# MayeulCassier/Matrix-Factorization-With-Comparison-Data

Measured on AMD Instinct MI355X. Metric: triplet-updates/sec, higher is better.
Workload: dtype f32

## Files before the change

matrix-factorization-with-comparison-data_amd/csrc/resident_kernel.h:

```cpp
#pragma once
#include "common.h"
#include "train_common.h"

namespace mfcd_detail {

typedef unsigned long long u64;

#define MFCD_LAMBDA_INLINE __attribute__((always_inline))

#ifdef MFCD_RES_STATS
#define RS_NOW() ((u64)__builtin_amdgcn_s_memtime())
#define RS_ADD(slot, val) rs_acc[slot] += (u64)(val)
#else
#define RS_NOW() ((u64)0)
#define RS_ADD(slot, val) ((void)0)
#endif

typedef const __attribute__((address_space(4))) float *ScalarTablePtr;
__device__ __forceinline__ StepScalars load_step_scalars(const StepScalars *table, int k)
{
    const ScalarTablePtr f = (ScalarTablePtr)(table + k);
    StepScalars s;
    s.neg_step_size = f[0];
    s.bc2_sqrt = f[1];
    s.inv_bc2_sqrt = f[2];
    s.pad = 0.0f;
    return s;
}


__device__ __forceinline__ u64 pack_granule(unsigned tag, float v)
{
    return ((u64)tag << 32) | (u64)__float_as_uint(v);
}

__device__ __forceinline__ u64 load_granule(const u64 *p)
{
    return __hip_atomic_load(p, __ATOMIC_RELAXED, __HIP_MEMORY_SCOPE_AGENT);
}

__device__ __forceinline__ void store_granule(u64 *p, unsigned tag, float v)
{
    __hip_atomic_store(p, pack_granule(tag, v), __ATOMIC_RELAXED, __HIP_MEMORY_SCOPE_AGENT);
}

struct RowMap {
    int n, m, c;
    __host__ __device__ int vrow_u(int u) const { return u < c ? 2 * u : 2 * c + (u - c); }
    __host__ __device__ int vrow_v(int i) const { return i < c ? 2 * i + 1 : 2 * c + (i - c); }
    __host__ __device__ int users_below(int x) const
    {
        if (x <= 2 * c) return (x + 1) >> 1;
        return n > c ? c + (x - 2 * c) : c;
    }
    __host__ __device__ int items_below(int x) const
    {
        if (x <= 2 * c) return x >> 1;
        return m > c ? c + (x - 2 * c) : c;
    }
    __host__ __device__ bool is_item(int vr) const { return vr < 2 * c ? (vr & 1) != 0 : m > n; }
    __host__ __device__ int table_row(int vr) const { return vr < 2 * c ? vr >> 1 : c + (vr - 2 * c); }
};
__host__ __device__ inline RowMap make_row_map(int n, int m)
{
    RowMap r;
    r.n = n; r.m = m; r.c = n < m ? n : m;
    return r;
}

constexpr int kEventCap = 64;
constexpr unsigned kEventNone = 0xFFFFFFF8u;
constexpr int kEventMaxLocalRows = 1024;

struct ResidentArgs {
    const ResidentCold *cold;
    const mfcd_sample *samples;
    const StepScalars *sc;
    u64 *mailbox;
    void *loss_terms;
    u64 *dbg;
    unsigned tag_base;
    int64_t N;
    int B, n, m, K, NW;
    int lookahead;
    int fast_math;
    int bf16;
    AdamStatic ac;
};

__device__ __forceinline__ mfcd_sample load_record(const mfcd_sample *__restrict__ samples, int64_t pos0, int Bk,
                                                   int base, int lane)
{
    mfcd_sample s;
    s.u = s.i = s.j = -0x40000000;
    s.z = 0.0f;
    if (base + lane < Bk) s = samples[pos0 + base + lane];
    return s;
}

struct Masks {
    u64 mu, mi, mj;
};

template <int D, int Q, int LOOK, bool FAST, bool BF16 = false>
__global__ __launch_bounds__(256) __attribute__((amdgpu_waves_per_eu(Q >= 16 ? 2 : 1)))
void resident_train_kernel(ResidentArgs a)
{
    constexpr int S = D >= 64 ? D / 64 : 1;
    constexpr int RPR = D < 64 ? 64 / D : 1;
    constexpr int EW = 64 * Q;
    static_assert(EW % D == 0, "a wave's slice must hold whole rows");
    static_assert(EW / D <= kEventMaxLocalRows, "local row indices are 10-bit fields of an event entry");
    constexpr bool GRL = Q >= 16;
    extern __shared__ __attribute__((aligned(16))) float lds_dyn[];
    const int lane = threadIdx.x & 63;
    const int gw = blockIdx.x * (blockDim.x >> 6) + (threadIdx.x >> 6);
    if (gw >= a.NW) return;

    const int64_t T = (int64_t)(a.n + a.m) * D;
    const int64_t ebase = (int64_t)gw * EW;
    const int Rlo = (int)(ebase / D);
    const int64_t eend = (ebase + EW < T) ? ebase + EW : T;
    const int Rhi = (int)(eend / D);
    const int lcol = lane & (D - 1);
    auto elem_is_item = [&](int64_t e) MFCD_LAMBDA_INLINE { return make_row_map(a.n, a.m).is_item((int)(e / D)); };
    auto elem_offset = [&](int64_t e) MFCD_LAMBDA_INLINE { return (int64_t)make_row_map(a.n, a.m).table_row((int)(e / D)) * D + (e % D); };

#ifdef MFCD_RES_STATS
    u64 rs_acc[8] = {0, 0, 0, 0, 0, 0, 0, 0};
    const u64 rs_t0 = RS_NOW();
    [[maybe_unused]] const u64 rs_abs_t0 = __builtin_amdgcn_s_memrealtime();
    [[maybe_unused]] u64 rs_abs_l0 = 0, rs_abs_l1 = 0;
    [[maybe_unused]] u64 rs_hit[8] = {0, 0, 0, 0, 0, 0, 0, 0};
    [[maybe_unused]] u64 rs_mark = 0;
#endif
    float p[Q], m1[Q], m2[Q], gr[GRL ? 1 : Q];
    float *const lgr = lds_dyn + (threadIdx.x >> 6) * (GRL ? EW : 0);
    auto post = [](float x) MFCD_LAMBDA_INLINE {
        if constexpr (BF16) return (float)(mfcd_bf16)x;
        else return x;
    };
    {
        const ResidentCold c = *a.cold;
#pragma unroll
        for (int q = 0; q < Q; ++q) {
            const int64_t e = ebase + q * 64 + lane;
            p[q] = m1[q] = m2[q] = 0.0f;
            if constexpr (GRL) lgr[q * 64 + lane] = 0.0f;
            if (e < T) {
                const int64_t o = elem_offset(e);
                if (!elem_is_item(e)) { p[q] = BF16 ? (float)((const mfcd_bf16 *)c.U)[o] : c.U[o]; m1[q] = c.mU[o]; m2[q] = c.vU[o]; }
                else { p[q] = BF16 ? (float)((const mfcd_bf16 *)c.V)[o] : c.V[o]; m1[q] = c.mV[o]; m2[q] = c.vV[o]; }
            }
        }
    }

    auto batch_size = [&](int step) MFCD_LAMBDA_INLINE {
        const int64_t pos0 = (int64_t)step * a.B;
        return (int)((a.N - pos0) < a.B ? (a.N - pos0) : a.B);
    };
    auto scan = [&](const mfcd_sample &s, int Bk, int base) MFCD_LAMBDA_INLINE {
        const bool valid = base + lane < Bk;
        const int ru = s.u, ri = s.i, rj = s.j;
        Masks M;
        M.mu = __ballot(valid && ru >= Rlo && ru < Rhi);
        M.mi = __ballot(valid && ri >= Rlo && ri < Rhi);
        M.mj = __ballot(valid && rj >= Rlo && rj < Rhi);
        return M;
    };
    auto reg_of = [&](int lr) MFCD_LAMBDA_INLINE { return D >= 64 ? lr * S : lr / RPR; };

    auto give_up = [&](int step, int64_t pos, int what) MFCD_LAMBDA_INLINE {
        int *const status = a.cold->status;
        if (lane == 0) {
            if (__hip_atomic_exchange(status, 1, __ATOMIC_RELAXED, __HIP_MEMORY_SCOPE_AGENT) == 0 && a.dbg) {
                a.dbg[0] = (u64)gw; a.dbg[1] = (u64)step; a.dbg[2] = (u64)pos; a.dbg[3] = (u64)what;
            }
        }
    };
    auto poll_failed = [&](unsigned &spins, unsigned &limit) MFCD_LAMBDA_INLINE -> bool {
        if (spins == 0) limit = (unsigned)a.cold->spin_limit;
        ++spins;
        if (spins > limit || (spins & 255u) == 0) {
            if (spins > limit ||
                __hip_atomic_load(a.cold->status, __ATOMIC_RELAXED, __HIP_MEMORY_SCOPE_AGENT) != 0)
                return true;
        }
        return false;
    };

    auto store_row = [&](int lr, int64_t slot, unsigned tag) MFCD_LAMBDA_INLINE {
        u64 *dst = a.mailbox + slot * D;
        const int q0 = reg_of(lr);
#pragma unroll
        for (int q = 0; q < Q; ++q) {
            if (q >= q0 && q < q0 + S) {
                if constexpr (D >= 64) {
                    store_granule(dst + (q - q0) * 64 + lane, tag, p[q]);
                } else {
                    if (lane / D == lr % RPR) store_granule(dst + lcol, tag, p[q]);
                }
            }
        }
    };

    auto process_hit = [&](bool own0, bool own1, bool own2, int lr0, int lr1, int lr2, float zz, int64_t pos,
                           unsigned tag, float inv_batch, int step) MFCD_LAMBDA_INLINE -> bool {
        const bool own[3] = {own0, own1, own2};
        const int lrs[3] = {lr0, lr1, lr2};
        const u64 *slot = a.mailbox + pos * 3 * D;

        float row[3][S];
#pragma unroll
        for (int r = 0; r < 3; ++r) {
#pragma unroll
            for (int s2 = 0; s2 < S; ++s2) row[r][s2] = 0.0f;
            if (!own[r]) continue;
            const int q0 = reg_of(lrs[r]);
            if constexpr (D >= 64) {
#pragma unroll
                for (int q = 0; q < Q; ++q)
                    if (q >= q0 && q < q0 + S) row[r][(q * 64 % D) / 64] = p[q];
            } else {
                float sel = 0.0f;
#pragma unroll
                for (int q = 0; q < Q; ++q) sel = (q == q0) ? p[q] : sel;
                const float v = __shfl(sel, (lrs[r] % RPR) * D + lcol, MFCD_WAVE);
                row[r][0] = lane < D ? v : 0.0f;
            }
        }
        unsigned spins = 0, limit = 0;
        [[maybe_unused]] u64 rs_w0 = 0;
        RS_ADD(4, 1ull);
#ifdef MFCD_RES_STAMPS
        { const u64 t = RS_NOW(); rs_hit[0] += t - rs_mark; rs_mark = t; }
#endif
#if defined(MFCD_RES_STAGGER) && MFCD_RES_STAGGER > 0
        {
            u64 ga[3][S], gb[3][S];
            auto issue = [&](u64 (&g)[3][S]) MFCD_LAMBDA_INLINE {
#pragma unroll
                for (int r = 0; r < 3; ++r) {
                    if (own[r]) continue;
#pragma unroll
                    for (int s2 = 0; s2 < S; ++s2) {
                        const int c = lane + 64 * s2;
                        if (c < D) g[r][s2] = load_granule(slot + (int64_t)r * D + c);
                    }
                }
            };
            auto check = [&](const u64 (&g)[3][S]) MFCD_LAMBDA_INLINE -> bool {
                bool ok = true;
#pragma unroll
                for (int r = 0; r < 3; ++r) {
                    if (own[r]) continue;
#pragma unroll
                    for (int s2 = 0; s2 < S; ++s2) {
                        const int c = lane + 64 * s2;
                        if (c < D) {
                            ok = ok && ((unsigned)(g[r][s2] >> 32) == tag);
                            row[r][s2] = __uint_as_float((unsigned)g[r][s2]);
                        }
                    }
                }
                return __all(ok);
            };
            issue(ga);
            if (!check(ga)) {
#ifdef MFCD_RES_STATS
                rs_w0 = RS_NOW();
#endif
                issue(ga);
                __builtin_amdgcn_s_sleep(MFCD_RES_STAGGER);
                issue(gb);
                while (true) {
                    RS_ADD(5, 1);
                    if (poll_failed(spins, limit)) {
                        give_up(step, pos, (own0 ? 1 : 0) | (own1 ? 2 : 0) | (own2 ? 4 : 0));
                        return false;
                    }
                    if (check(ga)) break;
                    issue(ga);
                    if (check(gb)) break;
                    issue(gb);
                }
            }
        }
#else
        while (true) {
            bool ok = true;
#pragma unroll
            for (int r = 0; r < 3; ++r) {
                if (own[r]) continue;
#pragma unroll
                for (int s2 = 0; s2 < S; ++s2) {
                    const int c = lane + 64 * s2;
                    if (c < D) {
                        const u64 gq = load_granule(slot + (int64_t)r * D + c);
                        ok = ok && ((unsigned)(gq >> 32) == tag);
                        row[r][s2] = __uint_as_float((unsigned)gq);
                    }
                }
            }
            if (__all(ok)) break;
#ifdef MFCD_RES_STATS
            if (spins == 0) rs_w0 = RS_NOW();
            RS_ADD(5, 1);
#endif
            if (poll_failed(spins, limit)) {
                give_up(step, pos, (own0 ? 1 : 0) | (own1 ? 2 : 0) | (own2 ? 4 : 0));
                return false;
            }
        }
#endif
#ifdef MFCD_RES_STATS
        if (spins) RS_ADD(2, RS_NOW() - rs_w0);
        else RS_ADD(4, 1ull << 40);
#endif
#ifdef MFCD_RES_STAMPS
        { const u64 t = RS_NOW(); rs_hit[1] += t - rs_mark; if (!spins) { rs_hit[6] += t - rs_mark; rs_hit[7] += 1; } rs_mark = t; }
#endif

        float acc = 0.0f;
#pragma unroll
        for (int s2 = 0; s2 < S; ++s2) acc += row[0][s2] * (row[1][s2] - row[2][s2]);
        float pr, g;
        if constexpr (FAST) {
            const float x = wave_sum64(acc);
            const float e = __builtin_amdgcn_exp2f(x * -1.44269504088896340736f);
            const float dn = 1.0f + e;
            pr = div_newton(1.0f, dn, __builtin_amdgcn_rcpf(dn));
            pr = (e == __builtin_inff()) ? 0.0f : pr;
            const float den = fmaxf((1.0f - pr) * pr, 1e-12f);
            const float num = inv_batch * (pr - zz);
            g = div_newton(num, den, __builtin_amdgcn_rcpf(den)) * (1.0f - pr) * pr;
        } else {
            pr = sigmoid_f32(wave_sum64(acc));
            g = bce_sigmoid_backward_f32(pr, zz, inv_batch);
        }
        if (own[0] && lane == 0) {
            if constexpr (LOOK > 0) store_granule((u64 *)a.loss_terms + pos, tag, pr);
            else ((float *)a.loss_terms)[pos] = pr;
        }

        float du[S], dv[S];
#pragma unroll
        for (int s2 = 0; s2 < S; ++s2) {
            du[s2] = g * (row[1][s2] - row[2][s2]);
            dv[s2] = g * row[0][s2];
        }
        if constexpr (D < 64) {
            du[0] = __shfl(du[0], lcol, MFCD_WAVE);
            dv[0] = __shfl(dv[0], lcol, MFCD_WAVE);
        }
        if constexpr (GRL) {
#pragma unroll
            for (int r = 0; r < 3; ++r) {
                if (!own[r]) continue;
                const int q0 = reg_of(lrs[r]);
                if constexpr (D >= 64) {
#pragma unroll
                    for (int s2 = 0; s2 < S; ++s2)
                        lgr[(q0 + s2) * 64 + lane] += r == 0 ? du[s2] : (r == 1 ? dv[s2] : -dv[s2]);
                } else {
                    if (lane / D == lrs[r] % RPR) lgr[q0 * 64 + lane] += r == 0 ? du[0] : (r == 1 ? dv[0] : -dv[0]);
                }
            }
        } else {
#pragma unroll
            for (int q = 0; q < Q; ++q) {
                const int rowq = (q * 64 + lane) / D;
                const int sq = D >= 64 ? (q * 64 % D) / 64 : 0;
                if (own[0] && rowq == lrs[0]) gr[q] += du[sq];
                if (own[1] && rowq == lrs[1]) gr[q] += dv[sq];
                if (own[2] && rowq == lrs[2]) gr[q] += -dv[sq];
            }
        }
#ifdef MFCD_RES_STAMPS
        { const u64 t = RS_NOW(); rs_hit[2] += t - rs_mark; rs_mark = t; }
#endif
        return true;
    };

    auto step_update = [&](bool hit, const StepScalars &sc) MFCD_LAMBDA_INLINE {
        if constexpr (GRL) {
            if (hit) {
#pragma unroll
                for (int q = 0; q < Q; ++q) {
                    const float g = lgr[q * 64 + lane];
                    lgr[q * 64 + lane] = 0.0f;
                    adam_update_t<FAST>(p[q], m1[q], m2[q], g, a.ac, sc);
                    p[q] = post(p[q]);
                }
            } else {
#pragma unroll
                for (int q = 0; q < Q; ++q) {
                    adam_update_t<FAST>(p[q], m1[q], m2[q], 0.0f, a.ac, sc);
                    p[q] = post(p[q]);
                }
            }
        } else {
            adam_update_q<FAST, Q, false>(p, m1, m2, gr, a.ac, sc);
            if constexpr (BF16) {
#pragma unroll
                for (int q = 0; q < Q; ++q) p[q] = post(p[q]);
            }
        }
    };

    auto generic_loop = [&]() MFCD_LAMBDA_INLINE -> bool {
        auto publish = [&](int step) MFCD_LAMBDA_INLINE {
            const int64_t pos0 = (int64_t)step * a.B;
            const int Bk = batch_size(step);
            for (int base = 0; base < Bk; base += MFCD_WAVE) {
                const mfcd_sample s = load_record(a.samples, pos0, Bk, base, lane);
                const Masks M = scan(s, Bk, base);
                u64 mask = M.mu | M.mi | M.mj;
                while (mask) {
                    const int tl = __ffsll((long long)mask) - 1;
                    mask &= mask - 1;
                    const int64_t slot0 = (pos0 + base + tl) * 3;
                    if ((M.mu >> tl) & 1ull) store_row(__shfl(s.u, tl, MFCD_WAVE) - Rlo, slot0 + 0, a.tag_base + (unsigned)step + 1u);
                    if ((M.mi >> tl) & 1ull) store_row(__shfl(s.i, tl, MFCD_WAVE) - Rlo, slot0 + 1, a.tag_base + (unsigned)step + 1u);
                    if ((M.mj >> tl) & 1ull) store_row(__shfl(s.j, tl, MFCD_WAVE) - Rlo, slot0 + 2, a.tag_base + (unsigned)step + 1u);
                }
            }
        };
        publish(0);
        for (int k = 0; k < a.K; ++k) {
            const int64_t pos0 = (int64_t)k * a.B;
            const int Bk = batch_size(k);
            const float inv_batch = 1.0f / (float)Bk;
            const StepScalars sc = load_step_scalars(a.sc, k);
            if constexpr (!GRL) {
#pragma unroll
                for (int q = 0; q < Q; ++q) gr[q] = 0.0f;
            }
            bool any_hit = false;
            for (int base = 0; base < Bk; base += MFCD_WAVE) {
                const mfcd_sample s = load_record(a.samples, pos0, Bk, base, lane);
                const Masks M = scan(s, Bk, base);
                u64 mask = M.mu | M.mi | M.mj;
                any_hit = any_hit || mask != 0ull;
                while (mask) {
                    const int tl = __ffsll((long long)mask) - 1;
                    mask &= mask - 1;
                    const int hu = __shfl(s.u, tl, MFCD_WAVE) - Rlo, hi = __shfl(s.i, tl, MFCD_WAVE) - Rlo,
                              hj = __shfl(s.j, tl, MFCD_WAVE) - Rlo;
                    const float hz = __shfl(s.z, tl, MFCD_WAVE);
                    const bool ok = process_hit((bool)((M.mu >> tl) & 1ull), (bool)((M.mi >> tl) & 1ull),
                                                (bool)((M.mj >> tl) & 1ull), hu, hi, hj, hz, pos0 + base + tl,
                                                a.tag_base + (unsigned)k + 1u, inv_batch, k);
                    if (__builtin_amdgcn_readfirstlane((int)!ok)) return false;
                }
            }
            step_update(any_hit, sc);
            if (k + 1 < a.K) publish(k + 1);
        }
        return true;
    };

    bool alive = true;

    if constexpr (LOOK > 0) {
        const int W = __builtin_amdgcn_readfirstlane(a.lookahead);
        const int N32 = (int)a.N;
        const int gws = __builtin_amdgcn_readfirstlane(gw);
        const int tshift = (int)a.cold->tshift;
        const int NCH = ((a.K - 1) >> tshift) + 1;

        bool fits = true;
        {
            const unsigned *cnt = a.cold->ev_cnt + (size_t)gws * (size_t)a.cold->nch_cap;
            for (int c = lane; c < NCH; c += MFCD_WAVE) fits = fits && cnt[c] < (unsigned)kEventCap;
            fits = __all(fits);
        }
        if (!__builtin_amdgcn_readfirstlane((int)fits)) {
            alive = generic_loop();
        } else {
            unsigned ekey = kEventNone, erow = 0u;
            int estep = 0x7FFFFF;
            float ez = 0.0f;
            int chunk_end = 0;

            auto load_chunk = [&](int c) MFCD_LAMBDA_INLINE {
                const ResidentCold *cz = a.cold;
                const size_t li = (size_t)gws * (size_t)cz->nch_cap + (size_t)c;
                const uint4 e = cz->ev_ent[li * kEventCap + lane];
                const unsigned n_raw = cz->ev_cnt[li];
                const unsigned n = (unsigned)__builtin_amdgcn_readfirstlane((int)n_raw);
                const unsigned key = (unsigned)lane < n ? e.x : kEventNone;
                unsigned rank = 0u;
                for (unsigned l = 0; l < n; ++l) {
                    const unsigned kl = (unsigned)__builtin_amdgcn_readlane((int)key, (int)l);
                    rank += kl < key ? 1u : 0u;
                }
                const int dest = (int)((unsigned)lane < n ? rank : (unsigned)lane) << 2;
                ekey = (unsigned)__builtin_amdgcn_ds_permute(dest, (int)key);
                erow = (unsigned)__builtin_amdgcn_ds_permute(dest, (int)e.y);
                ez = __builtin_bit_cast(float, __builtin_amdgcn_ds_permute(dest, (int)e.z));
                estep = (int)(ekey >> 9);
                const int ce = (c + 1) << tshift;
                chunk_end = ce < a.K ? ce : a.K;
            };
            auto step_at = [&](int i) MFCD_LAMBDA_INLINE -> int { return __builtin_amdgcn_readlane(estep, i); };
            auto lanes_in = [](int lo, int hi) MFCD_LAMBDA_INLINE -> u64 { return ((1ull << hi) - 1ull) & ~((1ull << lo) - 1ull); };
            auto rowmask = [&](int lr) MFCD_LAMBDA_INLINE -> u64 {
                const bool t = ((ekey & 1u) && (int)(erow & 1023u) == lr) ||
                               ((ekey & 2u) && (int)((erow >> 10) & 1023u) == lr) ||
                               ((ekey & 4u) && (int)((erow >> 20) & 1023u) == lr);
                return __ballot(t);
            };

            auto publish_entry = [&](int idx, int jbase, int conf_lo, int conf_hi, int touch_lo, int touch_hi,
                                     bool need_touch) MFCD_LAMBDA_INLINE {
                const unsigned key_l = (unsigned)__builtin_amdgcn_readlane((int)ekey, idx);
                const unsigned row_l = (unsigned)__builtin_amdgcn_readlane((int)erow, idx);
                const int ke = (int)(key_l >> 9);
                const int tl = (int)((key_l >> 3) & 63u);
#pragma unroll 1
                for (int r = 0; r < 3; ++r) {
                    if (!((key_l >> r) & 1u)) continue;
                    const int lr = (int)((row_l >> (10 * r)) & 1023u);
                    if (conf_lo < conf_hi || need_touch) {
                        const u64 rm = rowmask(lr);
                        if (rm & lanes_in(conf_lo, conf_hi)) continue;
                        if (need_touch && !(rm & lanes_in(touch_lo, touch_hi))) continue;
                    }
                    const int q0 = reg_of(lr);
                    float pp[S], mm1[S], mm2[S];
#pragma unroll
                    for (int s2 = 0; s2 < S; ++s2) pp[s2] = mm1[s2] = mm2[s2] = 0.0f;
#pragma unroll
                    for (int q = 0; q < Q; ++q) {
                        if (q >= q0 && q < q0 + S) {
                            const int s2 = D >= 64 ? (q * 64 % D) / 64 : 0;
                            pp[s2] = p[q];
                            mm1[s2] = m1[q];
                            mm2[s2] = m2[q];
                        }
                    }
                    StepScalars scb = load_step_scalars(a.sc, jbase + 1);
#pragma unroll 1
                    for (int st = jbase + 1; st < ke; ++st) {
                        const StepScalars scn = load_step_scalars(a.sc, st + 1);
#pragma unroll
                        for (int s2 = 0; s2 < S; ++s2) {
                            adam_update_t<FAST>(pp[s2], mm1[s2], mm2[s2], 0.0f, a.ac, scb);
                            pp[s2] = post(pp[s2]);
                        }
                        scb = scn;
                    }
                    u64 *dst = a.mailbox + (((int64_t)ke * a.B + tl) * 3 + r) * D;
                    const unsigned tag = a.tag_base + (unsigned)ke + 1u;
                    if constexpr (D >= 64) {
#pragma unroll
                        for (int s2 = 0; s2 < S; ++s2) store_granule(dst + s2 * 64 + lane, tag, pp[s2]);
                    } else {
                        if (lane / D == lr % RPR) store_granule(dst + lcol, tag, pp[0]);
                    }
                    RS_ADD(7, 1);
                }
            };
            auto publish_fresh = [&](int jbase, int lo, int hi, int touch_lo, int touch_hi) MFCD_LAMBDA_INLINE {
                if (lo >= hi) return;
                [[maybe_unused]] const u64 rs_p0 = RS_NOW();
                int g0 = lo, gstep = step_at(lo);
                for (int idx = lo; idx < hi; ++idx) {
                    const int st = step_at(idx);
                    if (st != gstep) { g0 = idx; gstep = st; }
                    publish_entry(idx, jbase, lo, g0, touch_lo, touch_hi, jbase >= 0);
                }
                RS_ADD(3, RS_NOW() - rs_p0);
            };
            load_chunk(0);
            int hc = 0, pc = __builtin_popcountll(__ballot(estep < W));
            publish_fresh(-1, 0, pc, 0, 0);
            int nh = step_at(0), np = step_at(pc);
            auto next_event = [&]() MFCD_LAMBDA_INLINE -> int {
                const int cp = np - W;
                const int e = nh < cp ? nh : cp;
                return e < chunk_end ? e : chunk_end;
            };
            int next_evt = next_event();

            ScalarTablePtr scp = (ScalarTablePtr)a.sc;
            auto load_scalars_at = [&](ScalarTablePtr f) MFCD_LAMBDA_INLINE {
                StepScalars x;
                x.neg_step_size = f[0];
                x.bc2_sqrt = f[1];
                x.inv_bc2_sqrt = f[2];
                x.pad = 0.0f;
                return x;
            };
            StepScalars sc_cur = load_scalars_at(scp);
            int chunk = 0;
#ifdef MFCD_RES_STATS
            const u64 rs_l0 = RS_NOW();
            rs_acc[6] = rs_l0 - rs_t0;
            rs_abs_l0 = __builtin_amdgcn_s_memrealtime();
#endif
            int k = 0;
            while (true) {
                const int kq = next_evt < a.K ? next_evt : a.K;
                while (k < kq) {
                    scp += 4;
                    const StepScalars sc_next = load_scalars_at(scp);
                    if constexpr (GRL) {
                        step_update(false, sc_cur);
                    } else {
#pragma unroll
                        for (int q = 0; q < Q; ++q) {
                            adam_update_t<FAST>(p[q], m1[q], m2[q], 0.0f, a.ac, sc_cur);
                            p[q] = post(p[q]);
                        }
                    }
                    sc_cur = sc_next;
                    ++k;
                }
                if (k >= a.K) break;
                scp += 4;
                const StepScalars sc_next = load_scalars_at(scp);
                if constexpr (!GRL) {
#pragma unroll
                    for (int q = 0; q < Q; ++q) gr[q] = 0.0f;
                }
                bool hit = false;
                int h0 = 0;
                {
                    __builtin_amdgcn_s_setprio(3);
                    [[maybe_unused]] const u64 rs_e0 = RS_NOW();
#ifdef MFCD_RES_STAMPS
                    rs_mark = rs_e0;
#endif
                    RS_ADD(7, 1ull << 32);
                    if (k == chunk_end) {
                        load_chunk(++chunk);
                        hc = 0;
                        nh = step_at(0);
                        pc = __builtin_popcountll(__ballot(estep < k + W));
                        np = step_at(pc);
                    }
                    if (np == k + W) {
                        [[maybe_unused]] const u64 rs_p0 = RS_NOW();
                        const int g0 = pc;
                        do {
                            publish_entry(pc, k - 1, hc, g0, 0, 0, false);
                            ++pc;
                            np = step_at(pc);
                        } while (np == k + W);
                        RS_ADD(3, RS_NOW() - rs_p0);
                    }
                    h0 = hc;
                    if (nh == k) {
                        hit = true;
                        const int bk = (N32 - k * a.B) < a.B ? (N32 - k * a.B) : a.B;
                        const float inv_batch = 1.0f / (float)bk;
                        const unsigned tag = a.tag_base + (unsigned)k + 1u;
                        do {
                            const unsigned key_l = (unsigned)__builtin_amdgcn_readlane((int)ekey, hc);
                            const unsigned row_l = (unsigned)__builtin_amdgcn_readlane((int)erow, hc);
                            const float z_l = __builtin_bit_cast(float, __builtin_amdgcn_readlane(__builtin_bit_cast(int, ez), hc));
                            const bool ok = process_hit((bool)(key_l & 1u), (bool)(key_l & 2u), (bool)(key_l & 4u),
                                                        (int)(row_l & 1023u), (int)((row_l >> 10) & 1023u),
                                                        (int)((row_l >> 20) & 1023u), z_l,
                                                        (int64_t)k * a.B + (int)((key_l >> 3) & 63u), tag, inv_batch, k);
                            if (__builtin_amdgcn_readfirstlane((int)!ok)) { alive = false; break; }
                            ++hc;
                            nh = step_at(hc);
                        } while (nh == k);
                        if (!alive) break;
                    }
                    next_evt = next_event();
                    if (!hit) __builtin_amdgcn_s_setprio(0);
                    RS_ADD(1, RS_NOW() - rs_e0);
                }
                step_update(hit, sc_cur);
#ifdef MFCD_RES_STAMPS
                if (hit) { const u64 t = RS_NOW(); rs_hit[3] += t - rs_mark; rs_mark = t; }
#endif
                if (__builtin_expect(hit, 0)) {
                    publish_fresh(k, hc, pc, h0, hc);
                    __builtin_amdgcn_s_setprio(0);
#ifdef MFCD_RES_STAMPS
                    { const u64 t = RS_NOW(); rs_hit[4] += t - rs_mark; rs_hit[5] += 1; }
#endif
                }
                sc_cur = sc_next;
                ++k;
            }
            __builtin_amdgcn_s_setprio(0);
#ifdef MFCD_RES_STATS
            rs_abs_l1 = __builtin_amdgcn_s_memrealtime();
            rs_acc[0] = RS_NOW() - rs_l0;
            rs_acc[6] |= (u64)__builtin_amdgcn_s_getreg((31 << 11) | 4) << 32;
            rs_acc[5] |= (u64)__builtin_amdgcn_s_getreg((31 << 11) | 20) << 32;
            if (lane == 0 && a.dbg)
                for (int x = 0; x < 8; ++x) a.dbg[8 + (int64_t)gw * 8 + x] = rs_acc[x];
#endif
        }

        {
            float *const loss_out = a.cold->loss_out;
            if (loss_out != nullptr) {
                for (int k = gws; k < a.K && alive; k += a.NW) {
                    const int64_t off = (int64_t)k * a.B;
                    const int b = (int)((a.N - off) < a.B ? (a.N - off) : a.B);
                    const unsigned tag = a.tag_base + (unsigned)k + 1u;
                    const float zz = lane < b ? a.samples[off + lane].z : 0.0f;
                    unsigned spins = 0, limit = 0;
                    float pr = 0.0f;
                    while (true) {
                        bool ok = true;
                        if (lane < b) {
                            const u64 gq = load_granule((const u64 *)a.loss_terms + off + lane);
                            ok = (unsigned)(gq >> 32) == tag;
                            pr = __uint_as_float((unsigned)gq);
                        }
                        if (__all(ok)) break;
                        __builtin_amdgcn_s_sleep(8);
                        if (poll_failed(spins, limit)) {
                            give_up(k, off, 8);
                            alive = false;
                            break;
                        }
                    }
                    if (!alive) break;
                    float acc = lane < b ? bce_term_f32(pr, zz) : 0.0f;
                    acc = wave_sum64(acc);
                    if (lane == 0) loss_out[k] = acc / (float)b;
                }
            }
        }
        {
            unsigned *const cnt = a.cold->ev_cnt + (size_t)gws * (size_t)a.cold->nch_cap;
            for (int c = lane; c < NCH; c += MFCD_WAVE) cnt[c] = 0u;
        }
    } else {
        alive = generic_loop();
    }

    const ResidentCold c = *a.cold;
#pragma unroll
    for (int q = 0; q < Q; ++q) {
        const int64_t e = ebase + q * 64 + lane;
        if (e < T) {
            const int64_t o = elem_offset(e);
            if (!elem_is_item(e)) {
                if constexpr (BF16) ((mfcd_bf16 *)c.U)[o] = (mfcd_bf16)p[q];
                else c.U[o] = p[q];
                c.mU[o] = m1[q]; c.vU[o] = m2[q];
            } else {
                if constexpr (BF16) ((mfcd_bf16 *)c.V)[o] = (mfcd_bf16)p[q];
                else c.V[o] = p[q];
                c.mV[o] = m1[q]; c.vV[o] = m2[q];
            }
        }
    }
#ifdef MFCD_RES_STAMPS
    if (lane == 0 && a.dbg) {
        u64 *const o = a.dbg + 8 + (int64_t)gw * 8;
        o[1] = rs_abs_t0; o[2] = rs_abs_l0; o[3] = rs_abs_l1; o[7] = __builtin_amdgcn_s_memrealtime();
        for (int x = 0; x < 8; ++x) o[4096 * 8 + x] = rs_hit[x];
    }
#endif
}

}
```

Before: 92.71 million.

## Prefetch mailbox rows before publishing and split Adam update around publish

Splits hit processing into an early issue step that loads the two foreign mailbox rows and a later finish step, so the mailbox loads are in flight while the wave publishes entries for step k+W. The publish-due-roles computation is rewritten to precompute a per-lane due mask with a cross-lane scan. In the non-GRL path, only the registers touched by the hit are Adam-updated before publishing and the rest afterwards, shortening the critical path to the publish. The costs are more register pressure from holding the prefetched granules, a scalar loop in due_roles, and a more complicated ordering that could be wrong.

```diff
diff --git a/matrix-factorization-with-comparison-data_amd/csrc/resident_kernel.h b/matrix-factorization-with-comparison-data_amd/csrc/resident_kernel.h
--- a/matrix-factorization-with-comparison-data_amd/csrc/resident_kernel.h
+++ b/matrix-factorization-with-comparison-data_amd/csrc/resident_kernel.h
@@ -204,11 +204,46 @@
         }
     };
 
-    auto process_hit = [&](bool own0, bool own1, bool own2, int lr0, int lr1, int lr2, float zz, int64_t pos,
-                           unsigned tag, float inv_batch, int step) MFCD_LAMBDA_INLINE -> bool {
-        const bool own[3] = {own0, own1, own2};
-        const int lrs[3] = {lr0, lr1, lr2};
-        const u64 *slot = a.mailbox + pos * 3 * D;
+    struct Hit {
+        bool own[3];
+        int lr[3];
+        float z;
+        int64_t pos;
+        int fa, fb, nf;
+        u64 ga[S], gb[S];
+    };
+    auto issue_look = [&](Hit &h) MFCD_LAMBDA_INLINE {
+        if (h.nf == 0) return;
+        const u64 *slot = a.mailbox + h.pos * 3 * D;
+#pragma unroll
+        for (int s2 = 0; s2 < S; ++s2) {
+            const int c = lane + 64 * s2;
+            h.ga[s2] = h.gb[s2] = 0ull;
+            if (c < D) {
+                h.ga[s2] = load_granule(slot + (int64_t)h.fa * D + c);
+                h.gb[s2] = load_granule(slot + (int64_t)h.fb * D + c);
+            }
+        }
+    };
+    auto make_hit = [&](bool own0, bool own1, bool own2, int lr0, int lr1, int lr2, float zz, int64_t pos) MFCD_LAMBDA_INLINE {
+        Hit h;
+        h.own[0] = own0; h.own[1] = own1; h.own[2] = own2;
+        h.lr[0] = lr0; h.lr[1] = lr1; h.lr[2] = lr2;
+        h.z = zz;
+        h.pos = pos;
+        h.fa = !own0 ? 0 : (!own1 ? 1 : 2);
+        h.fb = !own2 ? 2 : (!own1 ? 1 : 0);
+        h.nf = (own0 ? 0 : 1) + (own1 ? 0 : 1) + (own2 ? 0 : 1);
+        issue_look(h);
+        return h;
+    };
+
+    [[maybe_unused]] unsigned touched_q = 0u;
+    auto finish_hit = [&](Hit &h, unsigned tag, float inv_batch, int step) MFCD_LAMBDA_INLINE -> bool {
+        const bool(&own)[3] = h.own;
+        const int(&lrs)[3] = h.lr;
+        const float zz = h.z;
+        const int64_t pos = h.pos;
 
         float row[3][S];
 #pragma unroll
@@ -235,84 +270,40 @@
 #ifdef MFCD_RES_STAMPS
         { const u64 t = RS_NOW(); rs_hit[0] += t - rs_mark; rs_mark = t; }
 #endif
-#if defined(MFCD_RES_STAGGER) && MFCD_RES_STAGGER > 0
-        {
-            u64 ga[3][S], gb[3][S];
-            auto issue = [&](u64 (&g)[3][S]) MFCD_LAMBDA_INLINE {
-#pragma unroll
-                for (int r = 0; r < 3; ++r) {
-                    if (own[r]) continue;
-#pragma unroll
-                    for (int s2 = 0; s2 < S; ++s2) {
-                        const int c = lane + 64 * s2;
-                        if (c < D) g[r][s2] = load_granule(slot + (int64_t)r * D + c);
-                    }
-                }
-            };
-            auto check = [&](const u64 (&g)[3][S]) MFCD_LAMBDA_INLINE -> bool {
-                bool ok = true;
-#pragma unroll
-                for (int r = 0; r < 3; ++r) {
-                    if (own[r]) continue;
-#pragma unroll
-                    for (int s2 = 0; s2 < S; ++s2) {
-                        const int c = lane + 64 * s2;
-                        if (c < D) {
-                            ok = ok && ((unsigned)(g[r][s2] >> 32) == tag);
-                            row[r][s2] = __uint_as_float((unsigned)g[r][s2]);
-                        }
-                    }
-                }
-                return __all(ok);
-            };
-            issue(ga);
-            if (!check(ga)) {
+        auto look_ok = [&]() MFCD_LAMBDA_INLINE -> bool {
+            bool ok = true;
+#pragma unroll
+            for (int s2 = 0; s2 < S; ++s2)
+                if (lane + 64 * s2 < D) ok = ok && (unsigned)(h.ga[s2] >> 32) == tag && (unsigned)(h.gb[s2] >> 32) == tag;
+            return __all(ok);
+        };
+        if (h.nf != 0 && !look_ok()) {
 #ifdef MFCD_RES_STATS
-                rs_w0 = RS_NOW();
-#endif
-                issue(ga);
-                __builtin_amdgcn_s_sleep(MFCD_RES_STAGGER);
-                issue(gb);
-                while (true) {
-                    RS_ADD(5, 1);
-                    if (poll_failed(spins, limit)) {
-                        give_up(step, pos, (own0 ? 1 : 0) | (own1 ? 2 : 0) | (own2 ? 4 : 0));
-                        return false;
-                    }
-                    if (check(ga)) break;
-                    issue(ga);
-                    if (check(gb)) break;
-                    issue(gb);
-                }
-            }
-        }
-#else
-        while (true) {
-            bool ok = true;
-#pragma unroll
-            for (int r = 0; r < 3; ++r) {
-                if (own[r]) continue;
-#pragma unroll
-                for (int s2 = 0; s2 < S; ++s2) {
-                    const int c = lane + 64 * s2;
-                    if (c < D) {
-                        const u64 gq = load_granule(slot + (int64_t)r * D + c);
-                        ok = ok && ((unsigned)(gq >> 32) == tag);
-                        row[r][s2] = __uint_as_float((unsigned)gq);
-                    }
-                }
-            }
-            if (__all(ok)) break;
-#ifdef MFCD_RES_STATS
-            if (spins == 0) rs_w0 = RS_NOW();
+            rs_w0 = RS_NOW();
+#endif
+            const int what = (own[0] ? 1 : 0) | (own[1] ? 2 : 0) | (own[2] ? 4 : 0);
             RS_ADD(5, 1);
-#endif
             if (poll_failed(spins, limit)) {
-                give_up(step, pos, (own0 ? 1 : 0) | (own1 ? 2 : 0) | (own2 ? 4 : 0));
+                give_up(step, pos, what);
                 return false;
             }
-        }
-#endif
+            while (true) {
+                issue_look(h);
+                if (look_ok()) break;
+                RS_ADD(5, 1);
+                if (poll_failed(spins, limit)) {
+                    give_up(step, pos, what);
+                    return false;
+                }
+            }
+        }
+#pragma unroll
+        for (int r = 0; r < 3; ++r) {
+            if (own[r]) continue;
+#pragma unroll
+            for (int s2 = 0; s2 < S; ++s2)
+                if (lane + 64 * s2 < D) row[r][s2] = __uint_as_float((unsigned)(r == h.fa ? h.ga[s2] : h.gb[s2]));
+        }
 #ifdef MFCD_RES_STATS
         if (spins) RS_ADD(2, RS_NOW() - rs_w0);
         else RS_ADD(4, 1ull << 40);
@@ -375,6 +366,9 @@
                 if (own[1] && rowq == lrs[1]) gr[q] += dv[sq];
                 if (own[2] && rowq == lrs[2]) gr[q] += -dv[sq];
             }
+#pragma unroll
+            for (int r = 0; r < 3; ++r)
+                if (own[r]) touched_q |= ((1u << S) - 1u) << reg_of(lrs[r]);
         }
 #ifdef MFCD_RES_STAMPS
         { const u64 t = RS_NOW(); rs_hit[2] += t - rs_mark; rs_mark = t; }
@@ -448,9 +442,9 @@
                     const int hu = __shfl(s.u, tl, MFCD_WAVE) - Rlo, hi = __shfl(s.i, tl, MFCD_WAVE) - Rlo,
                               hj = __shfl(s.j, tl, MFCD_WAVE) - Rlo;
                     const float hz = __shfl(s.z, tl, MFCD_WAVE);
-                    const bool ok = process_hit((bool)((M.mu >> tl) & 1ull), (bool)((M.mi >> tl) & 1ull),
-                                                (bool)((M.mj >> tl) & 1ull), hu, hi, hj, hz, pos0 + base + tl,
-                                                a.tag_base + (unsigned)k + 1u, inv_batch, k);
+                    Hit h = make_hit((bool)((M.mu >> tl) & 1ull), (bool)((M.mi >> tl) & 1ull),
+                                     (bool)((M.mj >> tl) & 1ull), hu, hi, hj, hz, pos0 + base + tl);
+                    const bool ok = finish_hit(h, a.tag_base + (unsigned)k + 1u, inv_batch, k);
                     if (__builtin_amdgcn_readfirstlane((int)!ok)) return false;
                 }
             }
@@ -512,70 +506,92 @@
                 return __ballot(t);
             };
 
-            auto publish_entry = [&](int idx, int jbase, int conf_lo, int conf_hi, int touch_lo, int touch_hi,
-                                     bool need_touch) MFCD_LAMBDA_INLINE {
+            auto publish_row = [&](int lr, int jbase, int ke, int tl, int r) MFCD_LAMBDA_INLINE {
+                const int q0 = reg_of(lr);
+                float pp[S], mm1[S], mm2[S];
+#pragma unroll
+                for (int s2 = 0; s2 < S; ++s2) pp[s2] = mm1[s2] = mm2[s2] = 0.0f;
+#pragma unroll
+                for (int q = 0; q < Q; ++q) {
+                    if (q >= q0 && q < q0 + S) {
+                        const int s2 = D >= 64 ? (q * 64 % D) / 64 : 0;
+                        pp[s2] = p[q];
+                        mm1[s2] = m1[q];
+                        mm2[s2] = m2[q];
+                    }
+                }
+                StepScalars scb = load_step_scalars(a.sc, jbase + 1);
+#pragma unroll 1
+                for (int st = jbase + 1; st < ke; ++st) {
+                    const StepScalars scn = load_step_scalars(a.sc, st + 1);
+#pragma unroll
+                    for (int s2 = 0; s2 < S; ++s2) {
+                        adam_update_t<FAST>(pp[s2], mm1[s2], mm2[s2], 0.0f, a.ac, scb);
+                        pp[s2] = post(pp[s2]);
+                    }
+                    scb = scn;
+                }
+                u64 *dst = a.mailbox + (((int64_t)ke * a.B + tl) * 3 + r) * D;
+                const unsigned tag = a.tag_base + (unsigned)ke + 1u;
+                if constexpr (D >= 64) {
+#pragma unroll
+                    for (int s2 = 0; s2 < S; ++s2) store_granule(dst + s2 * 64 + lane, tag, pp[s2]);
+                } else {
+                    if (lane / D == lr % RPR) store_granule(dst + lcol, tag, pp[0]);
+                }
+                RS_ADD(7, 1);
+            };
+            auto publish_entry = [&](int idx, int jbase, int conf_lo, int conf_hi) MFCD_LAMBDA_INLINE {
                 const unsigned key_l = (unsigned)__builtin_amdgcn_readlane((int)ekey, idx);
                 const unsigned row_l = (unsigned)__builtin_amdgcn_readlane((int)erow, idx);
-                const int ke = (int)(key_l >> 9);
-                const int tl = (int)((key_l >> 3) & 63u);
 #pragma unroll 1
                 for (int r = 0; r < 3; ++r) {
                     if (!((key_l >> r) & 1u)) continue;
                     const int lr = (int)((row_l >> (10 * r)) & 1023u);
-                    if (conf_lo < conf_hi || need_touch) {
-                        const u64 rm = rowmask(lr);
-                        if (rm & lanes_in(conf_lo, conf_hi)) continue;
-                        if (need_touch && !(rm & lanes_in(touch_lo, touch_hi))) continue;
-                    }
-                    const int q0 = reg_of(lr);
-                    float pp[S], mm1[S], mm2[S];
-#pragma unroll
-                    for (int s2 = 0; s2 < S; ++s2) pp[s2] = mm1[s2] = mm2[s2] = 0.0f;
-#pragma unroll
-                    for (int q = 0; q < Q; ++q) {
-                        if (q >= q0 && q < q0 + S) {
-                            const int s2 = D >= 64 ? (q * 64 % D) / 64 : 0;
-                            pp[s2] = p[q];
-                            mm1[s2] = m1[q];
-                            mm2[s2] = m2[q];
-                        }
-                    }
-                    StepScalars scb = load_step_scalars(a.sc, jbase + 1);
+                    if (conf_lo < conf_hi && (rowmask(lr) & lanes_in(conf_lo, conf_hi))) continue;
+                    publish_row(lr, jbase, (int)(key_l >> 9), (int)((key_l >> 3) & 63u), r);
+                }
+            };
+            auto due_roles = [&](int touch_lo, int lo, int hi, bool all_touched) MFCD_LAMBDA_INLINE -> unsigned {
+                if (lo >= hi) return 0u;
+                const unsigned x0 = erow & 1023u, x1 = (erow >> 10) & 1023u, x2 = (erow >> 20) & 1023u;
+                unsigned touched = all_touched ? 7u : 0u, conflict = 0u;
+                for (int src = touch_lo; src < hi; ++src) {
+                    const unsigned key_s = (unsigned)__builtin_amdgcn_readlane((int)ekey, src);
+                    const unsigned row_s = (unsigned)__builtin_amdgcn_readlane((int)erow, src);
+                    const bool earlier = (int)(key_s >> 9) < estep;
+#pragma unroll
+                    for (int r = 0; r < 3; ++r) {
+                        if (!((key_s >> r) & 1u)) continue;
+                        const unsigned y = (row_s >> (10 * r)) & 1023u;
+                        const unsigned names = (x0 == y ? 1u : 0u) | (x1 == y ? 2u : 0u) | (x2 == y ? 4u : 0u);
+                        if (src < lo) touched |= names;
+                        else conflict |= earlier ? names : 0u;
+                    }
+                }
+                return (lane >= lo && lane < hi) ? (touched & ~conflict & ekey & 7u) : 0u;
+            };
+            auto publish_due = [&](int jbase, unsigned due) MFCD_LAMBDA_INLINE {
+                u64 dm = __ballot(due != 0u);
+                if (!dm) return;
+                [[maybe_unused]] const u64 rs_p0 = RS_NOW();
+                while (dm) {
+                    const int idx = __ffsll((long long)dm) - 1;
+                    dm &= dm - 1;
+                    const unsigned key_l = (unsigned)__builtin_amdgcn_readlane((int)ekey, idx);
+                    const unsigned row_l = (unsigned)__builtin_amdgcn_readlane((int)erow, idx);
+                    const unsigned due_l = (unsigned)__builtin_amdgcn_readlane((int)due, idx);
 #pragma unroll 1
-                    for (int st = jbase + 1; st < ke; ++st) {
-                        const StepScalars scn = load_step_scalars(a.sc, st + 1);
-#pragma unroll
-                        for (int s2 = 0; s2 < S; ++s2) {
-                            adam_update_t<FAST>(pp[s2], mm1[s2], mm2[s2], 0.0f, a.ac, scb);
-                            pp[s2] = post(pp[s2]);
-                        }
-                        scb = scn;
-                    }
-                    u64 *dst = a.mailbox + (((int64_t)ke * a.B + tl) * 3 + r) * D;
-                    const unsigned tag = a.tag_base + (unsigned)ke + 1u;
-                    if constexpr (D >= 64) {
-#pragma unroll
-                        for (int s2 = 0; s2 < S; ++s2) store_granule(dst + s2 * 64 + lane, tag, pp[s2]);
-                    } else {
-                        if (lane / D == lr % RPR) store_granule(dst + lcol, tag, pp[0]);
-                    }
-                    RS_ADD(7, 1);
-                }
-            };
-            auto publish_fresh = [&](int jbase, int lo, int hi, int touch_lo, int touch_hi) MFCD_LAMBDA_INLINE {
-                if (lo >= hi) return;
-                [[maybe_unused]] const u64 rs_p0 = RS_NOW();
-                int g0 = lo, gstep = step_at(lo);
-                for (int idx = lo; idx < hi; ++idx) {
-                    const int st = step_at(idx);
-                    if (st != gstep) { g0 = idx; gstep = st; }
-                    publish_entry(idx, jbase, lo, g0, touch_lo, touch_hi, jbase >= 0);
+                    for (int r = 0; r < 3; ++r) {
+                        if (!((due_l >> r) & 1u)) continue;
+                        publish_row((int)((row_l >> (10 * r)) & 1023u), jbase, (int)(key_l >> 9), (int)((key_l >> 3) & 63u), r);
+                    }
                 }
                 RS_ADD(3, RS_NOW() - rs_p0);
             };
             load_chunk(0);
             int hc = 0, pc = __builtin_popcountll(__ballot(estep < W));
-            publish_fresh(-1, 0, pc, 0, 0);
+            publish_due(-1, due_roles(0, 0, pc, true));
             int nh = step_at(0), np = step_at(pc);
             auto next_event = [&]() MFCD_LAMBDA_INLINE -> int {
                 const int cp = np - W;
@@ -626,7 +642,7 @@
                     for (int q = 0; q < Q; ++q) gr[q] = 0.0f;
                 }
                 bool hit = false;
-                int h0 = 0;
+                unsigned due = 0u;
                 {
                     __builtin_amdgcn_s_setprio(3);
                     [[maybe_unused]] const u64 rs_e0 = RS_NOW();
@@ -641,50 +657,79 @@
                         pc = __builtin_popcountll(__ballot(estep < k + W));
                         np = step_at(pc);
                     }
+                    auto hit_at = [&](int idx) MFCD_LAMBDA_INLINE {
+                        const unsigned key_l = (unsigned)__builtin_amdgcn_readlane((int)ekey, idx);
+                        const unsigned row_l = (unsigned)__builtin_amdgcn_readlane((int)erow, idx);
+                        const float z_l = __builtin_bit_cast(float, __builtin_amdgcn_readlane(__builtin_bit_cast(int, ez), idx));
+                        return make_hit((bool)(key_l & 1u), (bool)(key_l & 2u), (bool)(key_l & 4u), (int)(row_l & 1023u),
+                                        (int)((row_l >> 10) & 1023u), (int)((row_l >> 20) & 1023u), z_l,
+                                        (int64_t)k * a.B + (int)((key_l >> 3) & 63u));
+                    };
+                    hit = nh == k;
+                    Hit h;
+                    if (hit) h = hit_at(hc);
                     if (np == k + W) {
                         [[maybe_unused]] const u64 rs_p0 = RS_NOW();
                         const int g0 = pc;
                         do {
-                            publish_entry(pc, k - 1, hc, g0, 0, 0, false);
+                            publish_entry(pc, k - 1, hc, g0);
                             ++pc;
                             np = step_at(pc);
                         } while (np == k + W);
                         RS_ADD(3, RS_NOW() - rs_p0);
                     }
-                    h0 = hc;
-                    if (nh == k) {
-                        hit = true;
+                    if (hit) {
                         const int bk = (N32 - k * a.B) < a.B ? (N32 - k * a.B) : a.B;
                         const float inv_batch = 1.0f / (float)bk;
                         const unsigned tag = a.tag_base + (unsigned)k + 1u;
-                        do {
-                            const unsigned key_l = (unsigned)__builtin_amdgcn_readlane((int)ekey, hc);
-                            const unsigned row_l = (unsigned)__builtin_amdgcn_readlane((int)erow, hc);
-                            const float z_l = __builtin_bit_cast(float, __builtin_amdgcn_readlane(__builtin_bit_cast(int, ez), hc));
-                            const bool ok = process_hit((bool)(key_l & 1u), (bool)(key_l & 2u), (bool)(key_l & 4u),
-                                                        (int)(row_l & 1023u), (int)((row_l >> 10) & 1023u),
-                                                        (int)((row_l >> 20) & 1023u), z_l,
-                                                        (int64_t)k * a.B + (int)((key_l >> 3) & 63u), tag, inv_batch, k);
+                        touched_q = 0u;
+                        const int hend = hc + __builtin_popcountll(__ballot(estep == k));
+                        due = due_roles(hc, hend, pc, false);
+                        while (true) {
+                            const bool ok = finish_hit(h, tag, inv_batch, k);
                             if (__builtin_amdgcn_readfirstlane((int)!ok)) { alive = false; break; }
                             ++hc;
                             nh = step_at(hc);
-                        } while (nh == k);
+                            if (nh != k) break;
+                            h = hit_at(hc);
+                        }
                         if (!alive) break;
                     }
                     next_evt = next_event();
                     if (!hit) __builtin_amdgcn_s_setprio(0);
                     RS_ADD(1, RS_NOW() - rs_e0);
                 }
-                step_update(hit, sc_cur);
+                if (__builtin_expect(hit, 0)) {
+                    if constexpr (GRL) {
+                        step_update(true, sc_cur);
+                    } else {
+#pragma unroll
+                        for (int q = 0; q < Q; ++q) {
+                            if ((touched_q >> q) & 1u) {
+                                adam_update_t<FAST>(p[q], m1[q], m2[q], gr[q], a.ac, sc_cur);
+                                p[q] = post(p[q]);
+                            }
+                        }
+                    }
 #ifdef MFCD_RES_STAMPS
-                if (hit) { const u64 t = RS_NOW(); rs_hit[3] += t - rs_mark; rs_mark = t; }
-#endif
-                if (__builtin_expect(hit, 0)) {
-                    publish_fresh(k, hc, pc, h0, hc);
+                    { const u64 t = RS_NOW(); rs_hit[3] += t - rs_mark; rs_mark = t; }
+#endif
+                    publish_due(k, due);
                     __builtin_amdgcn_s_setprio(0);
 #ifdef MFCD_RES_STAMPS
                     { const u64 t = RS_NOW(); rs_hit[4] += t - rs_mark; rs_hit[5] += 1; }
 #endif
+                    if constexpr (!GRL) {
+#pragma unroll
+                        for (int q = 0; q < Q; ++q) {
+                            if (!((touched_q >> q) & 1u)) {
+                                adam_update_t<FAST>(p[q], m1[q], m2[q], gr[q], a.ac, sc_cur);
+                                p[q] = post(p[q]);
+                            }
+                        }
+                    }
+                } else {
+                    step_update(false, sc_cur);
                 }
                 sc_cur = sc_next;
                 ++k;
```

After: 92.24 million. About the same (-0.5%).
